# cvangysel/cuNVSM

Hardware: AMD Instinct MI355X
Metric: n-gram windows/sec (batch=51200, NVSM config) (higher is better)
Workload: dtype f32

## Files before the change

### cunvsm_amd/_lib.py

```python
import ctypes as C
import os
import re
import subprocess

_HERE = os.path.dirname(os.path.abspath(__file__))
_ROOT = os.path.dirname(_HERE)
_SO = os.environ.get("CUNVSM_AMD_LIB") or os.path.join(_HERE, "libcunvsm_amd.so")
_HEADER = os.path.join(_ROOT, "include", "cunvsm_amd.h")
_HOOKS_SO = os.path.join(_HERE, "libcunvsm_amd_testhooks.so")
_HOOKS_HEADER = os.path.join(_ROOT, "include", "cunvsm_amd_test_hooks.h")

TANH, HARD_TANH = 0, 1
SGD, ADAGRAD, ADAM = 0, 1, 2
ADAM_NONE, ADAM_SPARSE, ADAM_DENSE_UPDATE, ADAM_DENSE_UPDATE_DENSE_VARIANCE = 0, 1, 2, 3
SAMPLER_HOST_MINSTD, SAMPLER_DEVICE = 0, 1
SIM_COSINE, SIM_DOT = 0, 1
SPACE_WORDS, SPACE_PROJECTED_WORDS, SPACE_ENTITIES = 0, 1, 2
ACT_MODEL, ACT_IDENTITY = -1, -2
LEX_JM, LEX_DIRICHLET = 0, 1
NORM_STANDARDIZE, NORM_MINMAX, NORM_NONE = 0, 1, 2
LEXICAL_MAX_QUERY_TERMS = 1024
ENSEMBLE_MAX_TOP_K = 1024

STATUS = {0: "OK", 1: "INVALID_ARGUMENT", 2: "UNSUPPORTED", 3: "DEVICE", 4: "STATE", 5: "NO_DEVICE"}
# ... 84 lines not shown

class NvsmNeighborOptions(C.Structure):
    _fields_ = [
        ("space", C.c_int32), ("similarity", C.c_int32), ("top_k", C.c_int32), ("exclude_self", C.c_int32),
        ("bias_coefficient", C.c_float), ("activation", C.c_int32),
        ("reserved", C.c_int32 * 6),
    ]


class GemmEpilogueArgs(C.Structure):
    _fields_ = [
        ("kernel", C.c_int), ("b_layout", C.c_int), ("M", C.c_int), ("N", C.c_int), ("K", C.c_int),
        ("A", C.c_void_p), ("B", C.c_void_p), ("C", C.c_void_p), ("alpha", C.c_float), ("bias", C.c_void_p),
        ("colstats", C.c_void_p), ("rowsq", C.c_void_p), ("rowsq_scale", C.c_float),
        ("pre", C.c_void_p), ("mean", C.c_void_p), ("inv_std", C.c_void_p), ("sums", C.c_void_p), ("n_global", C.c_double),
        ("dbeta", C.c_void_p), ("dgamma", C.c_void_p), ("grad_bias", C.c_void_p),
        ("table", C.c_void_p), ("table_rows", C.c_int64), ("idx", C.c_void_p), ("wts", C.c_void_p), ("window", C.c_int),
        ("A_out", C.c_void_p), ("launched", C.POINTER(C.c_int)),
    ]


class TablePassArgs(C.Structure):
    _fields_ = [
        ("table", C.c_int), ("kind", C.c_int), ("rows", C.c_int64), ("dim", C.c_int),
        ("n", C.c_int64), ("keys", C.c_void_p), ("div", C.c_int), ("num_src", C.c_int64),
        ("X", C.c_void_p), ("coef", C.c_void_p), ("sq_src", C.c_void_p), ("src_scale", C.c_void_p),
        ("P", C.c_void_p), ("m", C.c_void_p), ("v", C.c_void_p), ("sc_in", C.c_void_p), ("sc_out", C.c_void_p),
        ("lr", C.c_float), ("lambda_", C.c_float), ("decay", C.c_float), ("bc", C.c_float), ("dense", C.c_int),
        ("wide", C.c_int), ("nt", C.c_int), ("max_entries", C.c_int64), ("adam", C.c_int),
        ("one_launch", C.c_int), ("chunk_order", C.c_int), ("fill_in_bounds", C.c_int), ("entry_walk_min", C.c_int64),
        ("prev_n", C.c_int64), ("prev_keys", C.c_void_p),
        ("path", C.POINTER(C.c_int)), ("chunk", C.POINTER(C.c_int)), ("num_chunks", C.POINTER(C.c_int)),
        ("max_chunks", C.POINTER(C.c_int)), ("max_chunks2", C.POINTER(C.c_int)), ("arrive_left", C.POINTER(C.c_int)),
    ]


class LossArgs(C.Structure):
    _fields_ = [
        ("B", C.c_int64), ("de", C.c_int), ("R", C.c_int), ("k", C.c_int),
        ("pre", C.c_void_p), ("bn", C.c_int), ("bn_sums", C.c_void_p), ("bn_n", C.c_double), ("bias", C.c_void_p),
        ("E", C.c_void_p), ("rows", C.c_int64), ("ids", C.c_void_p), ("inst_w", C.c_void_p),
        ("nonlinearity", C.c_int), ("clip_sigmoid", C.c_int), ("bias_negative_samples", C.c_int), ("l2_entity", C.c_int),
        ("b_global", C.c_double),
        ("stamp", C.c_void_p), ("decay", C.c_void_p), ("now", C.c_int), ("rows_for_dispatch", C.c_int64), ("repeats", C.c_int),
        ("proj", C.c_void_p), ("dy", C.c_void_p), ("coef", C.c_void_p), ("probs", C.c_void_p), ("pp", C.c_void_p),
        ("bn_mean", C.c_void_p), ("bn_inv_std", C.c_void_p), ("loss", C.c_void_p), ("colstats", C.c_void_p),
        ("plan", C.POINTER(C.c_int)), ("arrive_left", C.POINTER(C.c_int)),
    ]


ALLREDUCE_FN = C.CFUNCTYPE(C.c_int, C.POINTER(C.c_double), C.c_int64, C.c_void_p)


def library_path():
    return _SO


def build_library(force=False):
    if force or not os.path.exists(_SO):
        subprocess.check_call(["make", "-C", os.path.join(_HERE, "csrc"), "-j8"] + (["-B"] if force else []))
    return _SO


def _declared(header):
    with open(header) as f:
        src = f.read()
# ... 4 lines not shown
def abi_symbols():
    return _declared(_HEADER)


def hook_symbols():
    return _declared(_HOOKS_HEADER)


class _Library:

    def __init__(self, product):
        self.__dict__["product"] = product
        self.__dict__["hooks"] = None

    def __getattr__(self, name):
        try:
            return getattr(self.product, name)
        except AttributeError:
            if not name.startswith("nvsm_debug_"):
                raise
        if self.hooks is None:
            if not os.path.exists(_HOOKS_SO):
                raise AttributeError("%s lives in %s, which is missing (make -C cunvsm_amd/csrc)" % (name, _HOOKS_SO))
            H = C.CDLL(_HOOKS_SO, mode=C.RTLD_GLOBAL)
            vp, i64 = C.c_void_p, C.c_int64
            P = C.POINTER
            for hook, (res, args) in {
                "nvsm_debug_delay": (C.c_int, [vp, C.c_int]),
                "nvsm_debug_set_table_pass_form": (C.c_int, [C.c_int]),
                "nvsm_debug_neighbors_force_plain": (C.c_int, [C.c_int]),
                "nvsm_debug_gemm": (C.c_int, [C.c_int, C.c_int, C.c_int, C.c_int, vp, vp, vp]),
                "nvsm_debug_gemm_epilogue": (C.c_int, [P(GemmEpilogueArgs)]),
                "nvsm_debug_table_pass": (C.c_int, [P(TablePassArgs)]),
                "nvsm_debug_loss": (C.c_int, [P(LossArgs)]),
                "nvsm_debug_gemm_plan": (C.c_int, [C.c_int] * 7 + [P(C.c_int), P(C.c_uint)]),
                "nvsm_debug_rank_layout": (C.c_int, [i64] * 5 + [P(i64), P(i64)]),
                "nvsm_debug_gemm_time": (C.c_int, [C.c_int, C.c_int, C.c_int, C.c_int, C.c_int, C.c_int, P(C.c_float)]),
                "nvsm_debug_dt_time": (C.c_int, [C.c_int, C.c_int, C.c_int, C.c_int, C.c_int, C.c_int, P(C.c_float), P(C.c_float)]),
                "nvsm_debug_sort": (C.c_int, [i64, C.c_int, vp, vp, vp, C.c_int, P(C.c_float)]),
                "nvsm_debug_gather_mean": (C.c_int, [i64, C.c_int, vp, vp, vp, C.c_int, i64, vp]),
            }.items():
                fn = getattr(H, hook)
                fn.restype = res
                fn.argtypes = args
            self.__dict__["hooks"] = H
        return getattr(self.hooks, name)


_lib = None


def lib():
    global _lib
    if _lib is not None:
        return _lib
    if not os.path.exists(_SO):
        raise ImportError("%s is missing: run `python -c 'import __graft_entry__ as g; g.build()'` "
                          "(cunvsm_amd has no CPU fallback)" % _SO)
    try:
        import torch
    except Exception:
        pass
    L = C.CDLL(_SO, mode=C.RTLD_GLOBAL)
    vp, i64, cp = C.c_void_p, C.c_int64, C.c_char_p
    P = C.POINTER
    sig = {
# ... 71 lines not shown
```

### cunvsm_amd/csrc/kernels.h

```cpp
#pragma once

#include <hip/hip_runtime.h>
#include <hip/hip_ext.h>
#include <stdint.h>

#include <algorithm>
#include <cmath>

#include <stdexcept>
#include <string>

#include "tuning.h"

namespace cunvsm {

struct Error : std::runtime_error {
    int status;
    Error(int st, const std::string& what) : std::runtime_error(what), status(st) {}
};

void set_launch_events(hipEvent_t start, hipEvent_t stop);
hipEvent_t take_launch_events(hipEvent_t* start);
#define NVSM_LAUNCH(kernel, grid, block, shmem, stream, ...)                                                       \
    do {                                                                                                          \
// ... 223 lines not shown
    int* chunk_base;
    int* chunk_desc;
    int* chunk2_base;
    int* chunk2_desc;
    int* chunk_order;
    int* num_chunks;
    int* num_touched;
    int* touched;
    float* partial;
    float* partial_q;
    float* partial2;
    float* partial2_q;
    int* arrive_row;
    int* arrive2;
    int64_t n;
    int64_t rows;
    int max_chunks, max_chunks2;
    int chunk;
};
constexpr int kChunk = 64;
constexpr int kChunkSmall = 32;
constexpr int64_t kChunkSmallMaxEntries = 131072;
constexpr int kFan = 32;
inline int csr_chunk_entries(bool adam, int dim, int64_t n) {
    return (!adam && n <= kChunkSmallMaxEntries && dim <= 128) ? kChunkSmall : kChunk;
}
inline void csr_chunk_caps(bool adam, int dim, int64_t max_entries, int* max_chunks, int* max_chunks2) {
    int64_t c1 = 2 * max_entries / kChunk;
    if (!adam && dim <= 128) c1 = std::max<int64_t>(c1, 2 * std::min<int64_t>(max_entries, kChunkSmallMaxEntries) / kChunkSmall);
    *max_chunks = static_cast<int>(c1 + 2);
    *max_chunks2 = static_cast<int>(c1 / kFan + 2);
}

void launch_csr_build(const Csr& c, hipStream_t s, bool counters_cleared = false, int* order_key = nullptr);
void launch_chunk_order(const Csr& c, int* key_in, int* key_out, void* sort_temp, size_t sort_temp_bytes, hipStream_t s, bool keys_written = false);
inline int64_t csr_counter_ints(int64_t rows) { return (2 * rows + 3 + 63) / 64 * 64; }
bool row_pass_split(const Csr& c);
double table_split_ratio();

enum RowKind {
    ROW_SGD = 0,
    ROW_ADAGRAD_ENT = 1,
    ROW_ADAM_MV = 2,
    ROW_ADAM_SPARSE_ENT = 3,
    ROW_ADAM_DENSE = 4,
    ROW_ADAM_FULL = 5,
    ROW_SCALAR_ACC = 6
};
struct RowPassArgs {
    int table;
    int kind;
    const float* X;
    const float* wts;
    const float* coefs;
    const float* sq_src;
    const float* src_scale;
    uint32_t div;
    uint64_t div_magic;
    float* P; float* m; float* v;
    const float* sc_in;
    float* sc_out;
    int dim;
    float lr, decay, lambda;
    float one_m_b1, s_m, one_m_b2, s_v, bc, eps, c_reg;
    int dense;
    int max_blocks;
    int touched_only;
    int nt_p;
    int nt_m;
// ... 108 lines not shown
```

### cunvsm_amd/csrc/model.cpp

```cpp
#include "model.h"

#include <dlfcn.h>

#include <algorithm>
#include <cmath>
#include <cstdio>
#include <cstdlib>
#include <cstring>
#include <sstream>

namespace cunvsm {

struct RcclApi {
    void* handle = nullptr;
    typedef struct { char internal[128]; } UniqueId;
    int (*GetUniqueId)(UniqueId*) = nullptr;
    int (*CommInitRank)(void**, int, UniqueId, int) = nullptr;
    int (*AllReduce)(const void*, void*, size_t, int, int, void*, hipStream_t) = nullptr;
    int (*AllGather)(const void*, void*, size_t, int, void*, hipStream_t) = nullptr;
    int (*CommDestroy)(void*) = nullptr;
    int (*CommCount)(void*, int*) = nullptr;
    const char* (*GetErrorString)(int) = nullptr;
    static constexpr int kInt8 = 0, kFloat32 = 7, kFloat64 = 8, kSum = 0;

// ... 285 lines not shown
static int bits_for(int64_t n) {
    int b = 1;
    while ((int64_t(1) << b) < n) ++b;
    return b;
}

bool Model::table_decays_lazily(bool documents, int64_t rows, int dim, int64_t max_entries) const {
    const int method = cfg_.update_method, mode = cfg_.adam_mode;
    const bool sparse_adam = method == NVSM_ADAM && mode <= NVSM_ADAM_SPARSE;
    const bool decays = sparse_adam || (method != NVSM_ADAM && cfg_.regularization_lambda > 0.f);
    const double lazy_min_mb = tune_.lazy_min_mb >= 0.0 ? tune_.lazy_min_mb : (sparse_adam ? 96.0 : 384.0);
    const double state_mb = static_cast<double>(rows) * dim * sizeof(float) * (method == NVSM_ADAM ? 2.0 : 1.0) / 1048576.0;
    const int tab_mask = tune_.lazy_tables;
    return tune_.lazy_decay && decays && state_mb >= lazy_min_mb && ((tab_mask >> (documents ? 1 : 0)) & 1) &&
           static_cast<double>(rows) * table_split_ratio() >= static_cast<double>(max_entries);
}

void Model::alloc_table_csr(TableState& t, int64_t max_entries, bool chunk_order) {
    const int64_t rows = t.rows;
    const int dim = t.dim;
    const int method = cfg_.update_method;
    t.max_entries = max_entries;
    csr_chunk_caps(method == NVSM_ADAM, dim, max_entries, &t.max_chunks, &t.max_chunks2);
    for (int k = 0; k < t.idx_sets; ++k) {
        TableState::CsrIndex& x = t.idx[k];
        x.sorted_key.alloc(max_entries); x.sorted_entry.alloc(max_entries);
        x.csr_zeroed.alloc(csr_counter_ints(rows), true); x.chunk_base.alloc(rows, true);
        x.touched.alloc(std::min<int64_t>(rows, max_entries));
        x.chunk_desc.alloc(static_cast<size_t>(t.max_chunks) * 3, true);
        x.chunk2_base.alloc(rows, true);
        x.chunk2_desc.alloc(static_cast<size_t>(t.max_chunks2) * 2, true);
        if (chunk_order) x.chunk_order.alloc(t.max_chunks, true);
    }
    if (t.idx[0].chunk_order.p) { t.chunk_key.alloc(t.max_chunks, true); t.chunk_key_sorted.alloc(t.max_chunks, true); }
    t.partial.alloc(static_cast<size_t>(t.max_chunks) * dim);
    t.partial_q.alloc(t.max_chunks, true);
    t.partial2.alloc(static_cast<size_t>(t.max_chunks2) * dim);
    t.partial2_q.alloc(t.max_chunks2, true);
    t.arrive2.alloc(t.max_chunks2, true);
    t.sort_bits = bits_for(rows);
    t.sort_temp_bytes = sort_pairs_temp_bytes(max_entries, t.sort_bits);
    t.sort_temp.alloc(t.sort_temp_bytes, true);
}

void Model::alloc_table(TableState& t, int64_t rows, int dim, int64_t max_entries) {
    t.rows = rows; t.dim = dim; t.max_entries = max_entries;
    t.P.alloc(rows * dim, true);
    const int method = cfg_.update_method, mode = cfg_.adam_mode;
    if (method == NVSM_ADAGRAD) {
        t.sc[0].alloc(rows, true); t.sc[1].alloc(rows, true);
    } else if (method == NVSM_ADAM) {
        t.m.alloc(rows * dim, true);
        if (mode == NVSM_ADAM_DENSE_UPDATE_DENSE_VARIANCE) t.vfull.alloc(rows * dim, true);
        else { t.sc[0].alloc(rows, true); t.sc[1].alloc(rows, true); }
    }
    alloc_table_csr(t, max_entries, chunk_order_enabled() && max_entries >= 60 * 4096);
    t.arrive_row.alloc(rows, true);
    {
        const bool sparse_adam = method == NVSM_ADAM && mode <= NVSM_ADAM_SPARSE;
        t.lazy = table_decays_lazily(&t == &ents_, rows, dim, max_entries);
        t.lazy_scalar = sparse_adam || (method == NVSM_ADAGRAD && &t == &ents_);
        if (t.lazy) t.stamp.alloc(rows, true);
        for (float& d : t.decay_hist) d = 1.f;
    }
}

void Model::alloc_sums(SumsBufs& b, int colgroups, int contrib_cap, int width_cap) {
// ... 1060 lines not shown

Csr Model::csr_of(TableState& t, int64_t n) {
    Csr c{};
    TableState::CsrIndex& x = t.idx[t.idx_cur];
    c.sorted_key = x.sorted_key.p; c.sorted_entry = x.sorted_entry.p;
    c.row_begin = x.csr_zeroed.p; c.row_end = x.csr_zeroed.p + t.rows; c.chunk_base = x.chunk_base.p;
    c.chunk_desc = x.chunk_desc.p; c.num_chunks = x.csr_zeroed.p + 2 * t.rows;
    c.num_touched = c.num_chunks + 2; c.touched = x.touched.p;
    c.partial = t.partial.p; c.partial_q = t.partial_q.p;
    c.chunk2_base = x.chunk2_base.p; c.chunk2_desc = x.chunk2_desc.p; c.chunk_order = x.chunk_order.p;
    c.partial2 = t.partial2.p; c.partial2_q = t.partial2_q.p;
    c.arrive_row = t.arrive_row.p; c.arrive2 = t.arrive2.p;
    c.n = n; c.rows = t.rows; c.max_chunks = t.max_chunks; c.max_chunks2 = t.max_chunks2;
    c.chunk = chunk_entries(t, n);
    return c;
}

void Model::build_csr(TableState& t, const int* keys, int64_t n, hipStream_t s, int64_t n_pair_entries) {
    if (t.idx_sets > 1) t.idx_cur ^= 1;
    TableState::CsrIndex& x = t.idx[t.idx_cur];
    const int* vals = nullptr;
    if (n_pair_entries > 0 && &t == &words_) {
        const int64_t n_text = n - n_pair_entries;
        const int w = cfg_.window_size;
        launch_pair_entry_ids(term_vals_.p, n_text, n_text / w, w, n_pair_entries, s);
        vals = term_vals_.p;
    } else if (n_pair_entries > 0) {
        const int64_t n_text = n - n_pair_entries;
        launch_pair_entry_ids(pair_vals_[t.idx_cur].p, n_text, n_text / R_, R_, n_pair_entries, s);
        vals = pair_vals_[t.idx_cur].p;
    }
    sort_pairs(t.sort_temp.p, t.sort_temp_bytes, &t.sort_epoch, keys, x.sorted_key.p, vals, x.sorted_entry.p, n, t.sort_bits, err_host_, s,
               x.csr_zeroed.p, csr_counter_ints(t.rows));
    launch_csr_build(csr_of(t, n), s, n > 0, x.chunk_order.p ? t.chunk_key.p : nullptr);
    if (x.chunk_order.p) launch_chunk_order(csr_of(t, n), t.chunk_key.p, t.chunk_key_sorted.p, t.sort_temp.p, t.sort_temp_bytes, s, n > 0);
}

static int nt_mask() {
    return tuning().nt_mask;
}

void Model::lazy_refresh(TableState& t, const Csr* touched, hipStream_t s) {
    if (!t.lazy) return;
    LazyRefreshArgs r{};
    r.P = t.P.p; r.m = t.m.p;
    r.sc = t.lazy_scalar ? t.sc[0].p : nullptr;
    r.sc_snapshot = t.lazy_scalar ? t.sc[1].p : nullptr;
    r.stamp = t.stamp.p; r.rows = t.rows; r.dim = t.dim; r.now = t.updates_done;
    r.s_m = 1.f; r.s_v = 1.f;
    if (cfg_.update_method == NVSM_ADAM) { RowPassArgs c{}; fill_adam_consts(c, 1.f, 0.f); r.s_m = c.s_m; r.s_v = c.s_v; }
    std::memcpy(r.decay, t.decay_hist, sizeof(r.decay));
    int64_t max_rows = t.rows;
    if (touched) { r.list = touched->touched; r.list_count = touched->num_touched; max_rows = std::min<int64_t>(touched->n, t.rows); }
    PROF_ON(&t == &words_ ? "lazy_refresh_words" : "lazy_refresh_entities", s);
    launch_lazy_refresh(r, max_rows, s);
}

LazyView Model::lazy_view(const TableState& t) const {
    LazyView v{};
    if (!t.lazy) return v;
    v.stamp = t.stamp.p; v.now = t.updates_done;
    std::memcpy(v.decay, t.decay_hist, sizeof(v.decay));
    return v;
}

void Model::lazy_scalar_snapshot(TableState& t, const Csr& c, hipStream_t s) {
    if (!t.lazy || !t.lazy_scalar) return;
    LazyRefreshArgs r{};
// ... 959 lines not shown
```

### cunvsm_amd/csrc/model.h

```cpp
#pragma once

#include <cstdlib>
#include <hip/hip_runtime.h>

#include <cstdint>
#include <map>
#include <random>
#include <stdexcept>
#include <string>
#include <utility>
#include <vector>

#include "../../include/cunvsm_amd.h"
#include "kernels.h"

namespace cunvsm {

#define NVSM_HIP_CHECK(expr)                                                                         \
    do {                                                                                             \
        hipError_t _e = (expr);                                                                      \
        if (_e != hipSuccess)                                                                        \
            throw ::cunvsm::Error(NVSM_ERR_DEVICE, std::string(#expr) + ": " + hipGetErrorString(_e)); \
    } while (0)

// ... 31 lines not shown
    std::string only;
    void begin(const char* name, hipStream_t s);
    void end(hipStream_t s);
    bool bind(const char* name, hipEvent_t* start, hipEvent_t* stop);
    bool selected(const char* name) const;
    void note(const char* name) { if (enabled) ++notes_[name]; }
    void reset();
    std::vector<std::string> names() const;
    bool get(const std::string& name, double* ms, int64_t* launches);
    ~Profiler();
 private:
    struct Slot { std::vector<std::pair<hipEvent_t, hipEvent_t>> ev; size_t used = 0; };
    std::map<std::string, Slot> slots_;
    std::map<std::string, int64_t> notes_;
    Slot* cur_ = nullptr;
};

struct TableState {
    int64_t rows = 0;
    int dim = 0;
    DevBuf<float> P, m, vfull, sc[2];
    int sc_cur = 0;
    uint64_t t = 1;
    struct CsrIndex {
        DevBuf<int> sorted_key, sorted_entry, chunk_base, chunk_desc, chunk2_base, chunk2_desc;
        DevBuf<int> touched;
        DevBuf<int> chunk_order;
        DevBuf<int> csr_zeroed;
    };
    CsrIndex idx[2];
    int idx_sets = 1, idx_cur = 0;
    DevBuf<int> arrive_row, arrive2;
    DevBuf<float> partial, partial_q, partial2, partial2_q;
    DevBuf<int> chunk_key, chunk_key_sorted;
    DevBuf<char> sort_temp;
    size_t sort_temp_bytes = 0;
    uint64_t sort_epoch = 0;
    int sort_bits = 1;
    int max_chunks = 0, max_chunks2 = 0;
    int64_t max_entries = 0;
    bool lazy = false;
    bool lazy_scalar = false;
    DevBuf<int> stamp;
    int updates_done = 0;
    float decay_hist[kLazyHistory];
};

struct RankLayout { int64_t qn, S, ld, n_keys, npad; };
RankLayout rank_layout(int64_t rows, int64_t k, int64_t queries, int64_t score_floats, int64_t slab_cap = 0);
RankLayout rank_layout_candidates(const int64_t* offsets, int64_t queries);

class Model {
 public:
    explicit Model(const nvsm_config& cfg);
    ~Model();

    void initialize(uint64_t seed);
    void initialize_from_rng_state();
    uint64_t rng_get_state();
    void rng_set_state(uint64_t s);

    void compute_cost(const nvsm_batch& batch, const int64_t* entity_ids);
    void compute_gradients();
    void update(float lr, float scaled_lambda);
    float get_cost();
    double cost_f64() const { return cost_; }
    float scaled_regularization_lambda() const;
// ... 326 lines not shown
```

### cunvsm_amd/csrc/update.hip

```cpp
#include "kernels.h"
#include "device_utils.h"

#include <cstdlib>

namespace cunvsm {

__global__ void csr_bounds_kernel(const int* __restrict__ key, int64_t n, int* __restrict__ row_begin,
                                  int* __restrict__ row_end, int* __restrict__ touched, int* __restrict__ num_touched,
                                  int* __restrict__ chunk_base, int* __restrict__ chunk2_base, int* __restrict__ num_chunks, int chunk,
                                  int* __restrict__ chunk_desc, int* __restrict__ chunk2_desc, int max_chunks, int max_chunks2) {
    const int lane = threadIdx.x & 63;
    const uint64_t lt = (1ull << lane) - 1ull;
    for (int64_t i0 = blockIdx.x * static_cast<int64_t>(blockDim.x) + (threadIdx.x - lane); i0 < n;
         i0 += static_cast<int64_t>(gridDim.x) * blockDim.x) {
        const int64_t i = i0 + lane;
        const bool in = i < n;
        const int k = in ? key[i] : 0;
        const bool head = in && (i == 0 || key[i - 1] != k);
        if (head) row_begin[k] = static_cast<int>(i);
        const bool tail = in && (i == n - 1 || key[i + 1] != k);
        if (tail) row_end[k] = static_cast<int>(i + 1);
        uint64_t long_tails = __ballot(chunk_base && tail && i >= chunk && key[i - chunk] == k);
        while (long_tails) {
            const int l = __ffsll(static_cast<long long>(long_tails)) - 1;
            long_tails &= long_tails - 1;
            const int kk = __builtin_amdgcn_readlane(k, l);
            const int last = __builtin_amdgcn_readlane(static_cast<int>(i), l);
            int lo = 0, hi = last - chunk;
            while (lo < hi) {
                const int64_t span = hi - lo;
                const int p = lo + static_cast<int>(span * lane / 64);
                const int less = __popcll(__ballot(key[p] < kk));
                const int nlo = less == 0 ? lo : lo + static_cast<int>(span * (less - 1) / 64) + 1;
                const int nhi = less == 64 ? hi : lo + static_cast<int>(span * less / 64);
                lo = nlo; hi = nhi;
            }
            const int nch = (last + 1 - lo + chunk - 1) / chunk;
            int base = 0, base2 = 0;
            if (lane == l) {
                base = atomicAdd(num_chunks, nch);
                chunk_base[kk] = base;
                if (nch > kFan) { base2 = atomicAdd(num_chunks + 1, (nch + kFan - 1) / kFan); chunk2_base[kk] = base2; }
            }
            if (chunk_desc) {
                base = __shfl(base, l, 64); base2 = __shfl(base2, l, 64);
                for (int c = lane; c < nch; c += 64) {
                    if (base + c < max_chunks) {
                        const int first = lo + c * chunk;
                        chunk_desc[(base + c) * 3 + 0] = kk;
                        chunk_desc[(base + c) * 3 + 1] = first;
                        chunk_desc[(base + c) * 3 + 2] = min(last + 1, first + chunk);
                    }
                }
                if (nch > kFan) {
                    const int nch2 = (nch + kFan - 1) / kFan;
                    for (int c2 = lane; c2 < nch2; c2 += 64) {
                        if (base2 + c2 < max_chunks2) {
                            chunk2_desc[(base2 + c2) * 2 + 0] = base + c2 * kFan;
                            chunk2_desc[(base2 + c2) * 2 + 1] = base + min(nch, (c2 + 1) * kFan);
                        }
                    }
                }
            }
        }
        if (touched) {
            const uint64_t heads = __ballot(head);
            if (heads) {
                const int leader = __ffsll(static_cast<long long>(heads)) - 1;
                int base = 0;
                if (lane == leader) base = atomicAdd(num_touched, __popcll(heads));
                base = __shfl(base, leader, 64);
                if (head) touched[base + __popcll(heads & lt)] = k;
            }
        }
    }
}

__global__ void csr_chunks_kernel(const int* __restrict__ row_begin, const int* __restrict__ row_end, int64_t rows,
                                  int* __restrict__ chunk_base, int* __restrict__ chunk2_base, int* __restrict__ num_chunks, int chunk) {
    for (int64_t r = blockIdx.x * static_cast<int64_t>(blockDim.x) + threadIdx.x; r < rows;
         r += static_cast<int64_t>(gridDim.x) * blockDim.x) {
        const int cnt = row_end[r] - row_begin[r];
        if (cnt > chunk) {
            const int nch = (cnt + chunk - 1) / chunk;
            chunk_base[r] = atomicAdd(num_chunks, nch);
            if (nch > kFan) chunk2_base[r] = atomicAdd(num_chunks + 1, (nch + kFan - 1) / kFan);
        }
    }
}

__global__ void csr_chunk_fill_kernel(const int* __restrict__ key, int64_t n, const int* __restrict__ row_begin,
                                      const int* __restrict__ row_end, const int* __restrict__ chunk_base,
                                      const int* __restrict__ chunk2_base, int* __restrict__ chunk_desc,
                                      int* __restrict__ chunk2_desc, int max_chunks, int max_chunks2, const int* __restrict__ num_chunks,
                                      const int* __restrict__ sorted_entry, int* __restrict__ order_key, int chunk) {
    if (num_chunks[0] == 0) return;
    if (order_key) {
        const int nchunks = min(num_chunks[0], max_chunks);
        for (int ci = nchunks + blockIdx.x * blockDim.x + threadIdx.x; ci < max_chunks; ci += gridDim.x * blockDim.x) order_key[ci] = 511;
    }
    for (int64_t i = blockIdx.x * static_cast<int64_t>(blockDim.x) + threadIdx.x; i < n;
         i += static_cast<int64_t>(gridDim.x) * blockDim.x) {
        const int r = key[i];
        const int b = row_begin[r], e = row_end[r];
        const int cnt = e - b;
        const int rel = static_cast<int>(i) - b;
        if (cnt <= chunk || rel % chunk != 0) continue;
        const int c = rel / chunk;
        const int nch = (cnt + chunk - 1) / chunk;
        const int base = chunk_base[r];
        if (base + c < max_chunks) {
            chunk_desc[(base + c) * 3 + 0] = r;
            chunk_desc[(base + c) * 3 + 1] = static_cast<int>(i);
            chunk_desc[(base + c) * 3 + 2] = min(e, static_cast<int>(i) + chunk);
            if (order_key) {
                const uint64_t first = static_cast<uint32_t>(sorted_entry[i]);
                order_key[base + c] = static_cast<int>(min<uint64_t>(511, first * 512 / static_cast<uint64_t>(n)));
            }
        }
        if (nch > kFan && c % kFan == 0) {
            const int c2 = c / kFan;
            const int base2 = chunk2_base[r];
            if (base2 + c2 < max_chunks2) {
                chunk2_desc[(base2 + c2) * 2 + 0] = base + c;
                chunk2_desc[(base2 + c2) * 2 + 1] = base + min(nch, c + kFan);
            }
        }
    }
}

constexpr int64_t kCsrMergeMaxEntries = 64 * 4096;
static int csr_grid(int64_t items, bool sparse_table) {
    const int cap_env = tuning().csr_grid_cap;
    const int cap = cap_env >= 0 ? cap_env : (sparse_table ? 64 : 0);
    const int g = stream_grid(items, 256);
    return (cap > 0 && g > cap) ? cap : g;
}

void launch_csr_build(const Csr& c, hipStream_t s, bool counters_cleared, int* order_key) {
    const bool sparse = row_pass_split(c);
    if (!counters_cleared) (void)hipMemsetAsync(c.row_begin, 0, sizeof(int) * csr_counter_ints(c.rows), s);
    const bool reserve_in_bounds = c.n > 0 && c.n < kCsrMergeMaxEntries;
    const bool fill_in_bounds = reserve_in_bounds && !(c.chunk_order && order_key) && tuning().csr_fill_in_bounds;
    if (c.n > 0)
        hipLaunchKernelGGL(csr_bounds_kernel, dim3(csr_grid(c.n, sparse)), dim3(256), 0, s, c.sorted_key, c.n, c.row_begin, c.row_end,
                           row_pass_split(c) ? c.touched : nullptr, c.num_touched, reserve_in_bounds ? c.chunk_base : nullptr, c.chunk2_base, c.num_chunks, c.chunk,
                           fill_in_bounds ? c.chunk_desc : nullptr, c.chunk2_desc, c.max_chunks, c.max_chunks2);
    if (!reserve_in_bounds)
        hipLaunchKernelGGL(csr_chunks_kernel, dim3(csr_grid(c.rows, sparse)), dim3(256), 0, s, c.row_begin, c.row_end, c.rows,
                           c.chunk_base, c.chunk2_base, c.num_chunks, c.chunk);
    if (c.n > 0 && !fill_in_bounds)
        hipLaunchKernelGGL(csr_chunk_fill_kernel, dim3(csr_grid(c.n, sparse)), dim3(256), 0, s, c.sorted_key, c.n, c.row_begin,
                           c.row_end, c.chunk_base, c.chunk2_base, c.chunk_desc, c.chunk2_desc, c.max_chunks, c.max_chunks2, c.num_chunks,
                           c.sorted_entry, c.chunk_order ? order_key : nullptr, c.chunk);
}

#ifndef NVSM_SEG_UNROLL_WORDS
#define NVSM_SEG_UNROLL_WORDS 5
#endif
#ifndef NVSM_SEG_UNROLL_DOCS
#define NVSM_SEG_UNROLL_DOCS 5
#endif
template <int TABLE> struct SegUnrollDeep { static constexpr int value = TABLE == 0 ? NVSM_SEG_UNROLL_WORDS : NVSM_SEG_UNROLL_DOCS; };
#ifndef NVSM_SEG_UNROLL_WIDE_WORDS
#define NVSM_SEG_UNROLL_WIDE_WORDS 4
#endif
#ifndef NVSM_SEG_UNROLL_WIDE_DOCS
#define NVSM_SEG_UNROLL_WIDE_DOCS 3
#endif
template <int TABLE> struct SegUnrollWide { static constexpr int value = TABLE == 0 ? NVSM_SEG_UNROLL_WIDE_WORDS : NVSM_SEG_UNROLL_WIDE_DOCS; };
constexpr int kSegUnrollScalar = 4;
constexpr int kSegUnrollShallow = 3;

template <int V, int TABLE, bool VEC, int kSegUnroll = SegUnrollDeep<TABLE>::value>
__device__ __forceinline__ void accumulate_segment(const RowPassArgs& a, const int* __restrict__ sorted_entry,
                                                   int begin, int end, int col, float (&g)[V], float& q) {
#pragma clang fp contract(off)
    const bool need_q = (a.sq_src != nullptr);
    const int last = end - 1;
    int en_next[kSegUnroll];
#pragma unroll
    for (int u = 0; u < kSegUnroll; ++u) en_next[u] = sorted_entry[min(begin + u, last)];
    for (int e = begin; e < end; e += kSegUnroll) {
        uint32_t en[kSegUnroll];
#pragma unroll
        for (int u = 0; u < kSegUnroll; ++u) en[u] = static_cast<uint32_t>(en_next[u]);
        if (e + kSegUnroll < end) {
// ... 810 lines not shown
    if (cb_cap > 0 && chunk_blocks > cb_cap) chunk_blocks = cb_cap;
    if (a.rows_elsewhere && chunk_blocks > 2048) chunk_blocks = 2048;
    int64_t row_blocks = (row_items + gpb - 1) / gpb;
    { const int cap = tuning().row_blocks_cap; if (row_blocks > cap) row_blocks = cap; }
    if (a.max_blocks > 0 && row_blocks > a.max_blocks) row_blocks = a.max_blocks;
    if (row_blocks < 1) row_blocks = 1;
    if (a.rows_elsewhere) row_blocks = 0;
    if (chunk_blocks + row_blocks < 1) return;
    const dim3 grid(static_cast<unsigned>(chunk_blocks + row_blocks)), block(256);
#define NVSM_TABLE_LAUNCH(KERNEL, K, DEPTH) \
        if (a.rows_elsewhere) { \
            if (a.shallow) hipLaunchKernelGGL((KERNEL<V, TABLE, K, kSegUnrollShallow>), grid, block, 0, s, c, a, G, nvec, chunk_blocks); \
            else hipLaunchKernelGGL((KERNEL<V, TABLE, K, DEPTH<TABLE>::value>), grid, block, 0, s, c, a, G, nvec, chunk_blocks); \
        } else if (a.shallow) NVSM_LAUNCH((KERNEL<V, TABLE, K, kSegUnrollShallow>), grid, block, 0, s, c, a, G, nvec, chunk_blocks); \
        else NVSM_LAUNCH((KERNEL<V, TABLE, K, DEPTH<TABLE>::value>), grid, block, 0, s, c, a, G, nvec, chunk_blocks);
#define NVSM_TABLE_CASE(K) case K: NVSM_TABLE_LAUNCH(table_pass_kernel, K, SegUnrollDeep) break;
#define NVSM_TABLE_CASE_WIDE(K) case K: NVSM_TABLE_LAUNCH(table_pass_wide_kernel, K, SegUnrollWide) break;
    if (a.wide && a.kind == ROW_SGD) { NVSM_TABLE_LAUNCH(table_pass_wide_kernel, ROW_SGD, SegUnrollWide) return; }
    switch (a.kind) {
        NVSM_TABLE_CASE(ROW_SGD)
        NVSM_TABLE_CASE(ROW_ADAGRAD_ENT)
        NVSM_TABLE_CASE_WIDE(ROW_ADAM_MV)
        NVSM_TABLE_CASE_WIDE(ROW_ADAM_SPARSE_ENT)
        NVSM_TABLE_CASE_WIDE(ROW_ADAM_DENSE)
        NVSM_TABLE_CASE_WIDE(ROW_ADAM_FULL)
        NVSM_TABLE_CASE(ROW_SCALAR_ACC)
        default: break;
    }
#undef NVSM_TABLE_CASE_WIDE
#undef NVSM_TABLE_LAUNCH
#undef NVSM_TABLE_CASE
}

__global__ void chunk_order_key_kernel(Csr c, int* __restrict__ key) {
    const int nchunks = min(c.num_chunks[0], c.max_chunks);
    if (nchunks == 0) return;
    for (int ci = blockIdx.x * blockDim.x + threadIdx.x; ci < c.max_chunks; ci += gridDim.x * blockDim.x) {
        int k = 511;
        if (ci < nchunks) {
            const uint64_t e = static_cast<uint32_t>(c.sorted_entry[c.chunk_desc[ci * 3 + 1]]);
            k = static_cast<int>(min<uint64_t>(511, e * 512 / static_cast<uint64_t>(c.n)));
        }
        key[ci] = k;
    }
}
void launch_chunk_order(const Csr& c, int* key_in, int* key_out, void* sort_temp, size_t sort_temp_bytes, hipStream_t s, bool keys_written) {
    if (!c.chunk_order || c.n <= 0 || c.max_chunks <= 0) return;
    if (!keys_written) hipLaunchKernelGGL(chunk_order_key_kernel, dim3(stream_grid(c.max_chunks, 256)), dim3(256), 0, s, c, key_in);
    sort_pairs(sort_temp, sort_temp_bytes, nullptr, key_in, key_out, nullptr, c.chunk_order, c.max_chunks, 9, nullptr, s, nullptr, 0, c.num_chunks);
}

static bool entry_walk_enabled() {
    return tuning().entry_walk;
}
static int64_t entry_walk_min_entries(int table) {
    const Tuning& t = tuning();
    const long long per_table = table == 0 ? t.entry_walk_min_words : t.entry_walk_min_docs;
    return per_table >= 0 ? per_table : t.entry_walk_min;
}
static bool entry_walk_kind(int kind) { return kind == ROW_SGD || kind == ROW_ADAGRAD_ENT || kind == ROW_ADAM_MV || kind == ROW_ADAM_SPARSE_ENT; }

template <int V, int TABLE>
static void entry_walk_dispatch(const Csr& c, const RowPassArgs& a, int nvec, hipStream_t s) {
    if (c.n <= 0) return;
    int ppw = 16;
    while (ppw > 4 && c.n / ppw < 8192) ppw >>= 1;
    int64_t blocks = ((c.n + ppw - 1) / ppw + 3) / 4;
    if (blocks > 256 * 64) blocks = 256 * 64;
    const dim3 grid(static_cast<unsigned>(blocks)), block(256);
#define NVSM_WALK_CASE(K) case K: \
        if (nvec <= 64) NVSM_LAUNCH((entry_walk_kernel<V, TABLE, K, 1>), grid, block, 0, s, c, a, nvec, ppw); \
        else NVSM_LAUNCH((entry_walk_kernel<V, TABLE, K, 2>), grid, block, 0, s, c, a, nvec, ppw); \
        break;
    switch (a.kind) {
        NVSM_WALK_CASE(ROW_SGD)
        NVSM_WALK_CASE(ROW_ADAGRAD_ENT)
        NVSM_WALK_CASE(ROW_ADAM_MV)
        NVSM_WALK_CASE(ROW_ADAM_SPARSE_ENT)
        default: break;
    }
#undef NVSM_WALK_CASE
}

// ... 195 lines not shown
```

### include/cunvsm_amd_test_hooks.h

```cpp
#ifndef CUNVSM_AMD_TEST_HOOKS_H
#define CUNVSM_AMD_TEST_HOOKS_H

#include "cunvsm_amd.h"

#ifdef __cplusplus
extern "C" {
#endif

int nvsm_debug_gemm(int variant, int M, int N, int K, const float* hostA, const float* hostB, float* hostC);
enum { NVSM_DEBUG_GEMM_ROWS = 0, NVSM_DEBUG_GEMM_RSPLIT = 1, NVSM_DEBUG_GEMM_SPLIT = 2, NVSM_DEBUG_GEMM_TSTAT = 3,
       NVSM_DEBUG_GEMM_TILED = 4  };
typedef struct nvsm_debug_gemm_epilogue_args {
    int kernel, b_layout, M, N, K;
    const float* A;
    const float* B;
    float* C;
    float alpha;
    const float* bias;
    double* colstats;
    float* rowsq; float rowsq_scale;
    const float* pre; const float* mean; const float* inv_std; const double* sums; double n_global;
    float* dbeta; float* dgamma; float* grad_bias;
    const float* table; int64_t table_rows; const int64_t* idx; const float* wts; int window;
    float* A_out;
// ... 1 lines not shown
} nvsm_debug_gemm_epilogue_args;
int nvsm_debug_gemm_epilogue(const nvsm_debug_gemm_epilogue_args* args);
enum { NVSM_DEBUG_EPI_COLSTATS = 1, NVSM_DEBUG_EPI_ROWSQ = 2, NVSM_DEBUG_EPI_BN = 4, NVSM_DEBUG_EPI_BIAS = 8, NVSM_DEBUG_EPI_GATHER = 16,
       NVSM_DEBUG_EPI_BIAS_GRAD = 32 };
int nvsm_debug_gemm_plan(int kernel, int b_layout, int M, int N, int K, int flags, int window, int* covers, unsigned* plan);
int nvsm_debug_rank_layout(int64_t rows, int64_t k, int64_t queries, int64_t slab_mb, int64_t slab_cap, const int64_t* lengths, int64_t* out);
int nvsm_debug_delay(nvsm_model* m, int microseconds);
int nvsm_debug_set_table_pass_form(int one_launch);
typedef struct nvsm_debug_table_pass_args {
    int table;
    int kind;
    int64_t rows; int dim;
    int64_t n; const int32_t* keys;
    int div; int64_t num_src;
    const float* X;
    const float* coef;
    const float* sq_src;
    const float* src_scale;
    float* P; float* m; float* v;
    const float* sc_in; float* sc_out;
    float lr, lambda, decay, bc; int dense;
    int wide;
    int nt;
    int64_t max_entries; int adam;
    int one_launch, chunk_order, fill_in_bounds; int64_t entry_walk_min;
    int64_t prev_n; const int32_t* prev_keys;
    int* path;
    int* chunk;
    int* num_chunks;
    int* max_chunks; int* max_chunks2;
    int* arrive_left;
} nvsm_debug_table_pass_args;
int nvsm_debug_table_pass(const nvsm_debug_table_pass_args* args);
typedef struct nvsm_debug_loss_args {
    int64_t B; int de, R, k;
    const float* pre;
    int bn; const double* bn_sums;
    double bn_n; const float* bias;
    const float* E; int64_t rows;
    const int32_t* ids;
    const float* inst_w;
    int nonlinearity;
    int clip_sigmoid, bias_negative_samples, l2_entity;
    double b_global;
    const int32_t* stamp;
    const float* decay;
    int now;
    int64_t rows_for_dispatch;
    int repeats;
    float* proj; float* dy; float* coef; float* probs; float* pp; float* bn_mean; float* bn_inv_std;
    double* loss;
    double* colstats;
    int* plan;
    int* arrive_left;
} nvsm_debug_loss_args;
int nvsm_debug_loss(const nvsm_debug_loss_args* args);
int nvsm_debug_neighbors_force_plain(int on);
int nvsm_debug_gemm_time(int b_layout, int M, int N, int K, int extras, int repeats, float* avg_ms);
int nvsm_debug_dt_time(int M, int N, int rows, int slabs, int repeats, int which, float* kernel_ms, float* reduce_ms);
int nvsm_debug_sort(int64_t n, int bits, const int32_t* keys, int32_t* keys_out, int32_t* vals_out, int repeats, float* avg_ms);
int nvsm_debug_gather_mean(int64_t num_rows, int dim, const float* table, const int64_t* idx, const float* wts,
                           int window, int64_t num_out, float* out);

#ifdef __cplusplus
}
#endif
// ... 2 lines not shown
```

Before: 59.84 million.

## Replace chunk-order radix sort with in-build bucket histogram and counting scatter

```diff
diff --git a/cunvsm_amd/_lib.py b/cunvsm_amd/_lib.py
--- a/cunvsm_amd/_lib.py
+++ b/cunvsm_amd/_lib.py
@@ -140,6 +140,15 @@
         ("prev_n", C.c_int64), ("prev_keys", C.c_void_p),
         ("path", C.POINTER(C.c_int)), ("chunk", C.POINTER(C.c_int)), ("num_chunks", C.POINTER(C.c_int)),
         ("max_chunks", C.POINTER(C.c_int)), ("max_chunks2", C.POINTER(C.c_int)), ("arrive_left", C.POINTER(C.c_int)),
+    ]
+
+
+class ChunkOrderArgs(C.Structure):
+    _fields_ = [
+        ("rows", C.c_int64), ("dim", C.c_int), ("adam", C.c_int), ("n", C.c_int64), ("keys", C.c_void_p),
+        ("max_entries", C.c_int64), ("prev_n", C.c_int64), ("prev_keys", C.c_void_p),
+        ("chunk", C.POINTER(C.c_int)), ("num_chunks", C.POINTER(C.c_int)), ("max_chunks", C.POINTER(C.c_int)),
+        ("chunk_desc", C.c_void_p), ("order", C.c_void_p), ("sorted_entry", C.c_void_p), ("out_chunks", C.c_int64),
     ]
 
 
@@ -210,6 +219,7 @@
                 "nvsm_debug_gemm": (C.c_int, [C.c_int, C.c_int, C.c_int, C.c_int, vp, vp, vp]),
                 "nvsm_debug_gemm_epilogue": (C.c_int, [P(GemmEpilogueArgs)]),
                 "nvsm_debug_table_pass": (C.c_int, [P(TablePassArgs)]),
+                "nvsm_debug_chunk_order": (C.c_int, [P(ChunkOrderArgs)]),
                 "nvsm_debug_loss": (C.c_int, [P(LossArgs)]),
                 "nvsm_debug_gemm_plan": (C.c_int, [C.c_int] * 7 + [P(C.c_int), P(C.c_uint)]),
                 "nvsm_debug_rank_layout": (C.c_int, [i64] * 5 + [P(i64), P(i64)]),
diff --git a/cunvsm_amd/csrc/kernels.h b/cunvsm_amd/csrc/kernels.h
--- a/cunvsm_amd/csrc/kernels.h
+++ b/cunvsm_amd/csrc/kernels.h
@@ -279,9 +279,10 @@
     *max_chunks2 = static_cast<int>(c1 / kFan + 2);
 }
 
-void launch_csr_build(const Csr& c, hipStream_t s, bool counters_cleared = false, int* order_key = nullptr);
-void launch_chunk_order(const Csr& c, int* key_in, int* key_out, void* sort_temp, size_t sort_temp_bytes, hipStream_t s, bool keys_written = false);
-inline int64_t csr_counter_ints(int64_t rows) { return (2 * rows + 3 + 63) / 64 * 64; }
+void launch_csr_build(const Csr& c, hipStream_t s, bool counters_cleared = false);
+constexpr int kOrderBuckets = 512;
+inline int64_t csr_order_hist_offset(int64_t rows) { return (2 * rows + 3 + 63) / 64 * 64; }
+inline int64_t csr_counter_ints(int64_t rows) { return csr_order_hist_offset(rows) + 2 * kOrderBuckets + 4; }
 bool row_pass_split(const Csr& c);
 double table_split_ratio();
 
diff --git a/cunvsm_amd/csrc/model.cpp b/cunvsm_amd/csrc/model.cpp
--- a/cunvsm_amd/csrc/model.cpp
+++ b/cunvsm_amd/csrc/model.cpp
@@ -341,7 +341,6 @@
         x.chunk2_desc.alloc(static_cast<size_t>(t.max_chunks2) * 2, true);
         if (chunk_order) x.chunk_order.alloc(t.max_chunks, true);
     }
-    if (t.idx[0].chunk_order.p) { t.chunk_key.alloc(t.max_chunks, true); t.chunk_key_sorted.alloc(t.max_chunks, true); }
     t.partial.alloc(static_cast<size_t>(t.max_chunks) * dim);
     t.partial_q.alloc(t.max_chunks, true);
     t.partial2.alloc(static_cast<size_t>(t.max_chunks2) * dim);
@@ -1468,8 +1467,7 @@
     }
     sort_pairs(t.sort_temp.p, t.sort_temp_bytes, &t.sort_epoch, keys, x.sorted_key.p, vals, x.sorted_entry.p, n, t.sort_bits, err_host_, s,
                x.csr_zeroed.p, csr_counter_ints(t.rows));
-    launch_csr_build(csr_of(t, n), s, n > 0, x.chunk_order.p ? t.chunk_key.p : nullptr);
-    if (x.chunk_order.p) launch_chunk_order(csr_of(t, n), t.chunk_key.p, t.chunk_key_sorted.p, t.sort_temp.p, t.sort_temp_bytes, s, n > 0);
+    launch_csr_build(csr_of(t, n), s, n > 0);
 }
 
 static int nt_mask() {
diff --git a/cunvsm_amd/csrc/model.h b/cunvsm_amd/csrc/model.h
--- a/cunvsm_amd/csrc/model.h
+++ b/cunvsm_amd/csrc/model.h
@@ -87,7 +87,6 @@
     int idx_sets = 1, idx_cur = 0;
     DevBuf<int> arrive_row, arrive2;
     DevBuf<float> partial, partial_q, partial2, partial2_q;
-    DevBuf<int> chunk_key, chunk_key_sorted;
     DevBuf<char> sort_temp;
     size_t sort_temp_bytes = 0;
     uint64_t sort_epoch = 0;
diff --git a/cunvsm_amd/csrc/update.hip b/cunvsm_amd/csrc/update.hip
--- a/cunvsm_amd/csrc/update.hip
+++ b/cunvsm_amd/csrc/update.hip
@@ -4,11 +4,17 @@
 #include <cstdlib>
 
 namespace cunvsm {
+
+__device__ __forceinline__ int chunk_order_bucket(int first_entry, int64_t n) {
+    const uint64_t first = static_cast<uint32_t>(first_entry);
+    return static_cast<int>(min<uint64_t>(kOrderBuckets - 1, first * kOrderBuckets / static_cast<uint64_t>(n)));
+}
 
 __global__ void csr_bounds_kernel(const int* __restrict__ key, int64_t n, int* __restrict__ row_begin,
                                   int* __restrict__ row_end, int* __restrict__ touched, int* __restrict__ num_touched,
                                   int* __restrict__ chunk_base, int* __restrict__ chunk2_base, int* __restrict__ num_chunks, int chunk,
-                                  int* __restrict__ chunk_desc, int* __restrict__ chunk2_desc, int max_chunks, int max_chunks2) {
+                                  int* __restrict__ chunk_desc, int* __restrict__ chunk2_desc, int max_chunks, int max_chunks2,
+                                  const int* __restrict__ sorted_entry, int* __restrict__ order_hist) {
     const int lane = threadIdx.x & 63;
     const uint64_t lt = (1ull << lane) - 1ull;
     for (int64_t i0 = blockIdx.x * static_cast<int64_t>(blockDim.x) + (threadIdx.x - lane); i0 < n;
@@ -20,7 +26,9 @@
         if (head) row_begin[k] = static_cast<int>(i);
         const bool tail = in && (i == n - 1 || key[i + 1] != k);
         if (tail) row_end[k] = static_cast<int>(i + 1);
-        uint64_t long_tails = __ballot(chunk_base && tail && i >= chunk && key[i - chunk] == k);
+        const bool long_tail = (chunk_base || order_hist) && tail && i >= chunk && key[i - chunk] == k;
+        if (!chunk_base && long_tail) order_hist[2 * kOrderBuckets] = 1;
+        uint64_t long_tails = __ballot(chunk_base && long_tail);
         while (long_tails) {
             const int l = __ffsll(static_cast<long long>(long_tails)) - 1;
             long_tails &= long_tails - 1;
@@ -42,8 +50,12 @@
                 chunk_base[kk] = base;
                 if (nch > kFan) { base2 = atomicAdd(num_chunks + 1, (nch + kFan - 1) / kFan); chunk2_base[kk] = base2; }
             }
+            if (chunk_desc || order_hist) { base = __shfl(base, l, 64); base2 = __shfl(base2, l, 64); }
+            if (order_hist) {
+                for (int c = lane; c < nch; c += 64)
+                    if (base + c < max_chunks) atomicAdd(order_hist + chunk_order_bucket(sorted_entry[lo + c * chunk], n), 1);
+            }
             if (chunk_desc) {
-                base = __shfl(base, l, 64); base2 = __shfl(base2, l, 64);
                 for (int c = lane; c < nch; c += 64) {
                     if (base + c < max_chunks) {
                         const int first = lo + c * chunk;
@@ -77,7 +89,8 @@
 }
 
 __global__ void csr_chunks_kernel(const int* __restrict__ row_begin, const int* __restrict__ row_end, int64_t rows,
-                                  int* __restrict__ chunk_base, int* __restrict__ chunk2_base, int* __restrict__ num_chunks, int chunk) {
+                                  int* __restrict__ chunk_base, int* __restrict__ chunk2_base, int* __restrict__ num_chunks, int chunk,
+                                  const int* __restrict__ key, const int* __restrict__ sorted_entry, int64_t n, int* __restrict__ order_hist) {
     for (int64_t r = blockIdx.x * static_cast<int64_t>(blockDim.x) + threadIdx.x; r < rows;
          r += static_cast<int64_t>(gridDim.x) * blockDim.x) {
         const int cnt = row_end[r] - row_begin[r];
@@ -87,18 +100,42 @@
             if (nch > kFan) chunk2_base[r] = atomicAdd(num_chunks + 1, (nch + kFan - 1) / kFan);
         }
     }
+    if (!order_hist || !order_hist[2 * kOrderBuckets]) return;
+    for (int64_t i = blockIdx.x * static_cast<int64_t>(blockDim.x) + threadIdx.x; i < n;
+         i += static_cast<int64_t>(gridDim.x) * blockDim.x) {
+        const int r = key[i];
+        const int b = row_begin[r];
+        if (row_end[r] - b > chunk && (static_cast<int>(i) - b) % chunk == 0) atomicAdd(order_hist + chunk_order_bucket(sorted_entry[i], n), 1);
+    }
 }
 
 __global__ void csr_chunk_fill_kernel(const int* __restrict__ key, int64_t n, const int* __restrict__ row_begin,
                                       const int* __restrict__ row_end, const int* __restrict__ chunk_base,
                                       const int* __restrict__ chunk2_base, int* __restrict__ chunk_desc,
                                       int* __restrict__ chunk2_desc, int max_chunks, int max_chunks2, const int* __restrict__ num_chunks,
-                                      const int* __restrict__ sorted_entry, int* __restrict__ order_key, int chunk) {
+                                      const int* __restrict__ sorted_entry, int* __restrict__ chunk_order, int* __restrict__ order_hist,
+                                      int chunk) {
     if (num_chunks[0] == 0) return;
-    if (order_key) {
-        const int nchunks = min(num_chunks[0], max_chunks);
-        for (int ci = nchunks + blockIdx.x * blockDim.x + threadIdx.x; ci < max_chunks; ci += gridDim.x * blockDim.x) order_key[ci] = 511;
-    }
+    __shared__ int bucket_base[kOrderBuckets];
+    if (chunk_order) {
+        if (threadIdx.x < 64) {
+            constexpr int per_lane = kOrderBuckets / 64;
+            int cnt[per_lane], sum = 0;
+#pragma unroll
+            for (int j = 0; j < per_lane; ++j) { cnt[j] = order_hist[threadIdx.x * per_lane + j]; sum += cnt[j]; }
+            int incl = sum;
+#pragma unroll
+            for (int d = 1; d < 64; d <<= 1) {
+                const int up = __shfl_up(incl, d, 64);
+                if (static_cast<int>(threadIdx.x) >= d) incl += up;
+            }
+            int at = incl - sum;
+#pragma unroll
+            for (int j = 0; j < per_lane; ++j) { bucket_base[threadIdx.x * per_lane + j] = at; at += cnt[j]; }
+        }
+        __syncthreads();
+    }
+    int* const cursor = chunk_order ? order_hist + kOrderBuckets : nullptr;
     for (int64_t i = blockIdx.x * static_cast<int64_t>(blockDim.x) + threadIdx.x; i < n;
          i += static_cast<int64_t>(gridDim.x) * blockDim.x) {
         const int r = key[i];
@@ -113,9 +150,10 @@
             chunk_desc[(base + c) * 3 + 0] = r;
             chunk_desc[(base + c) * 3 + 1] = static_cast<int>(i);
             chunk_desc[(base + c) * 3 + 2] = min(e, static_cast<int>(i) + chunk);
-            if (order_key) {
-                const uint64_t first = static_cast<uint32_t>(sorted_entry[i]);
-                order_key[base + c] = static_cast<int>(min<uint64_t>(511, first * 512 / static_cast<uint64_t>(n)));
+            if (chunk_order) {
+                const int k = chunk_order_bucket(sorted_entry[i], n);
+                const int slot = bucket_base[k] + atomicAdd(cursor + k, 1);
+                if (static_cast<unsigned>(slot) < static_cast<unsigned>(max_chunks)) chunk_order[slot] = base + c;
             }
         }
         if (nch > kFan && c % kFan == 0) {
@@ -137,22 +175,24 @@
     return (cap > 0 && g > cap) ? cap : g;
 }
 
-void launch_csr_build(const Csr& c, hipStream_t s, bool counters_cleared, int* order_key) {
+void launch_csr_build(const Csr& c, hipStream_t s, bool counters_cleared) {
     const bool sparse = row_pass_split(c);
     if (!counters_cleared) (void)hipMemsetAsync(c.row_begin, 0, sizeof(int) * csr_counter_ints(c.rows), s);
+    int* const order_hist = c.chunk_order ? c.row_begin + csr_order_hist_offset(c.rows) : nullptr;
     const bool reserve_in_bounds = c.n > 0 && c.n < kCsrMergeMaxEntries;
-    const bool fill_in_bounds = reserve_in_bounds && !(c.chunk_order && order_key) && tuning().csr_fill_in_bounds;
+    const bool fill_in_bounds = reserve_in_bounds && !c.chunk_order && tuning().csr_fill_in_bounds;
     if (c.n > 0)
         hipLaunchKernelGGL(csr_bounds_kernel, dim3(csr_grid(c.n, sparse)), dim3(256), 0, s, c.sorted_key, c.n, c.row_begin, c.row_end,
                            row_pass_split(c) ? c.touched : nullptr, c.num_touched, reserve_in_bounds ? c.chunk_base : nullptr, c.chunk2_base, c.num_chunks, c.chunk,
-                           fill_in_bounds ? c.chunk_desc : nullptr, c.chunk2_desc, c.max_chunks, c.max_chunks2);
+                           fill_in_bounds ? c.chunk_desc : nullptr, c.chunk2_desc, c.max_chunks, c.max_chunks2, c.sorted_entry,
+                           order_hist);
     if (!reserve_in_bounds)
-        hipLaunchKernelGGL(csr_chunks_kernel, dim3(csr_grid(c.rows, sparse)), dim3(256), 0, s, c.row_begin, c.row_end, c.rows,
-                           c.chunk_base, c.chunk2_base, c.num_chunks, c.chunk);
+        hipLaunchKernelGGL(csr_chunks_kernel, dim3(std::max(csr_grid(c.rows, sparse), order_hist ? csr_grid(c.n, sparse) : 0)), dim3(256), 0, s,
+                           c.row_begin, c.row_end, c.rows, c.chunk_base, c.chunk2_base, c.num_chunks, c.chunk, c.sorted_key, c.sorted_entry, c.n, order_hist);
     if (c.n > 0 && !fill_in_bounds)
         hipLaunchKernelGGL(csr_chunk_fill_kernel, dim3(csr_grid(c.n, sparse)), dim3(256), 0, s, c.sorted_key, c.n, c.row_begin,
                            c.row_end, c.chunk_base, c.chunk2_base, c.chunk_desc, c.chunk2_desc, c.max_chunks, c.max_chunks2, c.num_chunks,
-                           c.sorted_entry, c.chunk_order ? order_key : nullptr, c.chunk);
+                           c.sorted_entry, c.chunk_order, order_hist, c.chunk);
 }
 
 #ifndef NVSM_SEG_UNROLL_WORDS
@@ -1029,23 +1069,6 @@
 #undef NVSM_TABLE_CASE
 }
 
-__global__ void chunk_order_key_kernel(Csr c, int* __restrict__ key) {
-    const int nchunks = min(c.num_chunks[0], c.max_chunks);
-    if (nchunks == 0) return;
-    for (int ci = blockIdx.x * blockDim.x + threadIdx.x; ci < c.max_chunks; ci += gridDim.x * blockDim.x) {
-        int k = 511;
-        if (ci < nchunks) {
-            const uint64_t e = static_cast<uint32_t>(c.sorted_entry[c.chunk_desc[ci * 3 + 1]]);
-            k = static_cast<int>(min<uint64_t>(511, e * 512 / static_cast<uint64_t>(c.n)));
-        }
-        key[ci] = k;
-    }
-}
-void launch_chunk_order(const Csr& c, int* key_in, int* key_out, void* sort_temp, size_t sort_temp_bytes, hipStream_t s, bool keys_written) {
-    if (!c.chunk_order || c.n <= 0 || c.max_chunks <= 0) return;
-    if (!keys_written) hipLaunchKernelGGL(chunk_order_key_kernel, dim3(stream_grid(c.max_chunks, 256)), dim3(256), 0, s, c, key_in);
-    sort_pairs(sort_temp, sort_temp_bytes, nullptr, key_in, key_out, nullptr, c.chunk_order, c.max_chunks, 9, nullptr, s, nullptr, 0, c.num_chunks);
-}
 
 static bool entry_walk_enabled() {
     return tuning().entry_walk;
diff --git a/include/cunvsm_amd_test_hooks.h b/include/cunvsm_amd_test_hooks.h
--- a/include/cunvsm_amd_test_hooks.h
+++ b/include/cunvsm_amd_test_hooks.h
@@ -57,6 +57,20 @@
     int* arrive_left;
 } nvsm_debug_table_pass_args;
 int nvsm_debug_table_pass(const nvsm_debug_table_pass_args* args);
+typedef struct nvsm_debug_chunk_order_args {
+    int64_t rows; int dim; int adam;
+    int64_t n; const int32_t* keys;
+    int64_t max_entries;
+    int64_t prev_n; const int32_t* prev_keys;
+    int* chunk;
+    int* num_chunks;
+    int* max_chunks;
+    int32_t* chunk_desc;
+    int32_t* order;
+    int32_t* sorted_entry;
+    int64_t out_chunks;
+} nvsm_debug_chunk_order_args;
+int nvsm_debug_chunk_order(const nvsm_debug_chunk_order_args* args);
 typedef struct nvsm_debug_loss_args {
     int64_t B; int de, R, k;
     const float* pre;
```

Result: slower. 58.52 million (-2.2%).
